# tho-kn/EgoTAP

Measured on AMD Instinct MI355X. Metric: stereo frames/sec (2D->3D lift, B=256, 256x256), higher is better.
Workload: dtype f32; 1 GPU; UnrealEgo 16-joint lifting head (heatmaps [B,90,64,64] -> joints [B,16,3]), forward only, fp32, batch 256 per GPU, inputs resident in HBM; batch_per_gpu=256, global_batch=256, heatmap=64, parallelism=dp1 (batch shards, no collective)

## Files before the change

egotap_amd/csrc/attention_f32.h:

```cpp
#pragma once
#include "common.h"
#include <math.h>
#ifdef EGOTAP_ATTN_F32_OLD
#include "../../tools/experiments/attention_f32_r2.h"
#else

template <int NW>
struct AttnCfg {
    static constexpr int DH = 128, KT = 32, KLD = DH + 4, THREADS = 64 * NW;
    static constexpr int TILE_FLOATS = KT * KLD + KT * DH;
    static constexpr int OUT_FLOATS = NW * 32 * KLD;
    static constexpr int LDS_BYTES = 4 * (TILE_FLOATS > OUT_FLOATS ? TILE_FLOATS : OUT_FLOATS);
};

template <int NW>
__global__ __launch_bounds__(64 * NW, 2) void attention_f32_kernel(const float* __restrict__ QKV,
                                                                 float* __restrict__ CTX, int N, int heads,
                                                                 int qgroups, float scale_log2e, float* __restrict__ LSE, int ksplit) {
    using Cfg = AttnCfg<NW>;
    constexpr int DH = Cfg::DH, KT = Cfg::KT, KLD = Cfg::KLD, THREADS = Cfg::THREADS;
    extern __shared__ __attribute__((aligned(16))) float smem[];
    float* Ks = smem;
    float* Vs = smem + KT * KLD;

    const int nblk = gridDim.x, bid = blockIdx.x;
    const int q8 = nblk >> 3, r8 = nblk & 7, x8 = bid & 7;
    const int lin = (x8 < r8 ? x8 * (q8 + 1) : r8 * (q8 + 1) + (x8 - r8) * q8) + (bid >> 3);
    const int split = ksplit > 1 ? lin % ksplit : 0;
    const int lq = ksplit > 1 ? lin / ksplit : lin;
    const int bh = lq / qgroups, qg = lq - bh * qgroups;
    const int b = bh / heads, h = bh - b * heads;

    const int tid = threadIdx.x, lane = tid & 63, wid = tid >> 6;
    const int l31 = lane & 31, lh = lane >> 5;
    const int D = heads * DH;
    const long ld = 3L * D;
    const float* base = QKV + (long)b * N * ld + h * DH;
    const int qb = qg * NW + wid;
    const bool valid = qb * 32 < N;
    const int q0 = min(qb * 32, N - 32);

    float qreg[64];
    {
        const float* qp = base + (long)(q0 + l31) * ld + 4 * lh;
#pragma unroll
        for (int t = 0; t < 16; ++t) {
            const f32x4 v = *(const f32x4*)(qp + 8 * t);
            qreg[4 * t + 0] = v[0]; qreg[4 * t + 1] = v[1]; qreg[4 * t + 2] = v[2]; qreg[4 * t + 3] = v[3];
        }
    }
    float m_run = -INFINITY, l_run = 0.f;

    constexpr int PER = KT * (DH / 4) / THREADS;
    f32x4 stg[PER];
    auto tile_req = [&](int kt, int vpart) __attribute__((always_inline)) {
        const float* kp = base + (long)min(kt * KT, N - KT) * ld + D + vpart * D;
#pragma unroll
        for (int i = 0; i < PER; ++i) {
            const int idx = tid + i * THREADS, row = idx >> 5, c4 = idx & 31;
            stg[i] = *(const f32x4*)(kp + (size_t)(unsigned)(row * (int)ld + c4 * 4));
        }
    };
    auto tile_put = [&](int vpart) __attribute__((always_inline)) {
#pragma unroll
        for (int i = 0; i < PER; ++i) {
            const int idx = tid + i * THREADS, row = idx >> 5, c4 = idx & 31;
            if (vpart) *(f32x4*)(Vs + row * DH + c4 * 4) = stg[i];
// ... 73 lines not shown
                s[r] = __builtin_amdgcn_exp2f(fmaf(s[r], scale_log2e, -m_run));
                psum += s[r];
            }
            l_run += psum;
#pragma unroll
            for (int r = 0; r < 16; ++r) {
                const float* vf = Vs + ((r & 3) + 8 * (r >> 2) + 4 * lh) * DH + l31;
#pragma unroll
                for (int dt = 0; dt < 4; ++dt)
                    o[dt] = __builtin_amdgcn_mfma_f32_32x32x2f32(vf[dt * 32], s[r], o[dt], 0, 0, 0);
            }
        }
        __syncthreads();
        if (kt + 1 < ntiles) {
            tile_put(1);
            if (kt + 2 < ntiles) tile_req(kt + 2, 0);
        }
    }
    __syncthreads();
    if (valid) {
        const float l_tot = l_run + __shfl_xor(l_run, 32, 64);
        const float inv = 1.0f / l_tot;
        const long part = ksplit > 1 ? (long)split * (gridDim.x / (ksplit * qgroups)) : 0;
        if (LSE != nullptr && lh == 0) LSE[(part + (long)b * heads + h) * N + q0 + l31] = m_run * 0.6931471805599453f + logf(l_tot);
        float* Os = smem + wid * 32 * KLD;
#pragma unroll
        for (int dt = 0; dt < 4; ++dt)
#pragma unroll
            for (int g = 0; g < 4; ++g) {
                f32x4 v;
#pragma unroll
                for (int c = 0; c < 4; ++c) v[c] = o[dt][4 * g + c] * inv;
                *(f32x4*)(Os + l31 * KLD + dt * 32 + 8 * g + 4 * lh) = v;
            }
        float* out = CTX + (part / heads * N + (long)b * N + q0) * D + h * DH;
#pragma unroll
        for (int it = 0; it < 16; ++it) {
            const int row = it * 2 + lh;
            const f32x4 v = *(const f32x4*)(Os + row * KLD + l31 * 4);
            *(f32x4*)(out + (long)row * D + l31 * 4) = v;
        }
    }
}

static __global__ __launch_bounds__(256) void attention_f32_merge_kernel(const float* __restrict__ part, const float* __restrict__ lse_part, float* __restrict__ ctx,
                                                                         int B, int N, int heads, int ksplit) {
    const long i = (long)blockIdx.x * blockDim.x + threadIdx.x;
    const long total = (long)B * N * heads * 32;
    if (i >= total) return;
    const int c4 = (int)(i & 31);
    const long t = i >> 5;
    const int h = (int)(t % heads);
    const long bn = t / heads;
    const int b = (int)(bn / N), n = (int)(bn - (long)b * N);
    float l[8], m = -INFINITY;
    for (int sp = 0; sp < ksplit; ++sp) {
        l[sp] = lse_part[(((long)sp * B + b) * heads + h) * N + n];
        m = fmaxf(m, l[sp]);
    }
    float wsum = 0.f;
    for (int sp = 0; sp < ksplit; ++sp) {
        l[sp] = expf(l[sp] - m);
        wsum += l[sp];
    }
    const float inv = 1.0f / wsum;
    f32x4 acc{0.f, 0.f, 0.f, 0.f};
    const long D = (long)heads * 128, off = bn * D + h * 128 + c4 * 4;
    for (int sp = 0; sp < ksplit; ++sp) {
        const f32x4 v = *(const f32x4*)(part + (long)sp * B * N * D + off);
        const float w = l[sp] * inv;
        acc[0] += w * v[0]; acc[1] += w * v[1]; acc[2] += w * v[2]; acc[3] += w * v[3];
    }
    *(f32x4*)(ctx + off) = acc;
}

static hipError_t attention_f32_launch(const float* QKV, float* CTX, int B, int N, int heads, hipStream_t stream,
                                       float* LSE = nullptr, float* scratch = nullptr, size_t scratch_floats = 0, int num_cu = 256) {
    constexpr int NW = 2;
    using Cfg = AttnCfg<NW>;
    if (B <= 0) return hipSuccess;
    if (N < 32 || N % 4 != 0) return hipErrorInvalidValue;
    auto kern = attention_f32_kernel<NW>;
    const int qgroups = ((N + 31) / 32 + NW - 1) / NW;
    const float scale_log2e = 1.4426950408889634f / sqrtf(128.0f);
    const long wgs = (long)B * heads * qgroups;
    int ksplit = 1;
    if (scratch != nullptr && LSE == nullptr) {
        const int ntiles = (N + 31) / 32;
        for (int k = 8; k >= 2; --k)
            if (ntiles % k == 0 && wgs * k <= 9L * num_cu / 2 && (size_t)k * ((size_t)B * N * heads * 128 + (size_t)B * heads * N) <= scratch_floats) { ksplit = k; break; }
    }
    if (ksplit > 1) {
        float* part = scratch;
        float* lse_part = scratch + (size_t)ksplit * B * N * heads * 128;
        hipLaunchKernelGGL(kern, dim3((unsigned)(wgs * ksplit)), dim3(Cfg::THREADS), Cfg::LDS_BYTES, stream, QKV, part, N, heads, qgroups, scale_log2e, lse_part, ksplit);
        hipError_t e = hipGetLastError();
        if (e != hipSuccess) return e;
        const long total = (long)B * N * heads * 32;
        hipLaunchKernelGGL(attention_f32_merge_kernel, dim3((unsigned)((total + 255) / 256)), dim3(256), 0, stream, (const float*)part, (const float*)lse_part, CTX, B, N, heads, ksplit);
        return hipGetLastError();
    }
    hipLaunchKernelGGL(kern, dim3(B * heads * qgroups), dim3(Cfg::THREADS), Cfg::LDS_BYTES, stream, QKV, CTX, N, heads,
                       qgroups, scale_log2e, LSE, 1);
    return hipGetLastError();
}
#endif
```

egotap_amd/csrc/egotap_abi.hip:

```cpp
#include <stdarg.h>
#include <stdio.h>
#include <string.h>

#include <string>
#include <unordered_map>
#include <vector>

#include "attention_f32.h"
#include "common.h"
#include "conv_f32.h"
#include "conv_bf16.h"
#include "gemm_f32.h"
#include "gemm_bf16.h"
#include "gemm_bf16_dma.h"
#include "gemm_f32_dma.h"
#include "attention_bf16.h"
#include "layernorm.h"
#include "metrics.h"
#include "heatmap_synth.h"
#include "pu_chain.h"
#include "gemm_tn_bf16.h"
#include "train_ops.h"
#include "gemm_bf16s.h"
#include "gemm_bf16s64.h"
// ... 407 lines not shown
    GemmTimer(Handle* h_, hipStream_t s_, const char* role, const char* kernel, double flops)
        : h(h_), s(s_), on(h_ && h_->timing) {
        if (!on) return;
        if (h->ev_used + 2 > h->ev.size()) {
            hipEvent_t a, b;
            if (hipEventCreate(&a) != hipSuccess || hipEventCreate(&b) != hipSuccess) { on = false; return; }
            h->ev.push_back(a);
            h->ev.push_back(b);
        }
        (void)hipEventRecord(h->ev[h->ev_used], s);
        h->rec.push_back({role, kernel, flops});
    }
    ~GemmTimer() {
        if (!on) return;
        (void)hipEventRecord(h->ev[h->ev_used + 1], s);
        h->ev_used += 2;
    }
};

template <class AL> struct AlName;
template <> struct AlName<ALoadPlain> { static constexpr const char* v = "ALoadPlain"; };
template <> struct AlName<ALoadPatch> { static constexpr const char* v = "ALoadPatch"; };
template <> struct AlName<ALoadTokens> { static constexpr const char* v = "ALoadTokens"; };
template <> struct AlName<ALoadRot> { static constexpr const char* v = "ALoadRot"; };
template <> struct AlName<ALoadStereo> { static constexpr const char* v = "ALoadStereo"; };
template <> struct AlName<ALoadStereoGated> { static constexpr const char* v = "ALoadStereoGated"; };
template <class E> struct EpiName;
template <> struct EpiName<EpiBias> { static constexpr const char* v = "EpiBias"; };
template <> struct EpiName<EpiBiasRes> { static constexpr const char* v = "EpiBiasRes"; };
template <> struct EpiName<EpiBiasGelu> { static constexpr const char* v = "EpiBiasGelu"; };
template <> struct EpiName<EpiBnLrelu> { static constexpr const char* v = "EpiBnLrelu"; };
template <> struct EpiName<EpiPatch> { static constexpr const char* v = "EpiPatch"; };

template <class Cfg, class AL, class Epi>
static hipError_t gemm(Handle* h, const char* role, const AL& al, const SegMat& W, const Epi& epi, float* C, long ldc,
                       int M, int N, int K, hipStream_t s) {
    static const std::string kname = std::string("gemm_f32_kernel<") + std::to_string(Cfg::BM) + "x" +
                                     std::to_string(Cfg::BN) + "x" + std::to_string(Cfg::BK) + "," + AlName<AL>::v + "," +
                                     EpiName<Epi>::v + ">";
    GemmTimer t(h, s, role, kname.c_str(), 2.0 * M * N * K);
    return gemm_f32_launch<Cfg, AL, Epi>(al, W, epi, C, ldc, M, N, K, s);
}

static int device_cu_count() {
    static int n = 0;
    if (n == 0) {
        int dev = 0, v = 0;
        if (hipGetDevice(&dev) == hipSuccess && hipDeviceGetAttribute(&v, hipDeviceAttributeMultiprocessorCount, dev) == hipSuccess && v > 0) n = v;
        else n = 256;
    }
    return n;
}
// ... 317 lines not shown
}

#if EGOTAP_IN(0)
static hipError_t gemm_res_ln(Handle* h, const char* role, const float* A, long lda, const float* Wp, const float* bias, float* X, int M, int D, int K,
                              const float* ln_g, const float* ln_b, float* Y, float* P, hipStream_t s) {
    if (D == 1024) {
        const SmallRoute r = gemm_small_route(h, true, M, D, K, D, device_cu_count());
        if ((r.kind == GS_SPLIT_S || r.kind == GS_SPLIT_A) && r.splits > 1) {
            static const std::string kname = "gemm_f32_splitk_kernel<ALoadPlain>+splitk_reduce_res_ln_kernel";
            GemmTimer t(h, s, role, kname.c_str(), 2.0 * M * D * K);
            hipError_t e = r.kind == GS_SPLIT_S ? gemm_f32_splitk_partials<TileS>(ALoadPlain{A, lda}, segmat1(Wp, D, K), P, SPLITK_FLOATS, M, D, K, s, r.splits)
                                                : gemm_f32_splitk_partials<TileA>(ALoadPlain{A, lda}, segmat1(Wp, D, K), P, SPLITK_FLOATS, M, D, K, s, r.splits);
            if (e != hipSuccess) return e;
            hipLaunchKernelGGL(splitk_reduce_res_ln_kernel<1024>, dim3(min((M + 3) / 4, 256 * 8)), dim3(256), 0, s, (const float*)P, bias, (const float*)X, X, ln_g,
                               ln_b, Y, M, r.splits, 1e-12f);
            return hipGetLastError();
        }
    }
    hipError_t e = gemm_small(h, role, ALoadPlain{A, lda}, segmat1(Wp, D, K), EpiBiasRes{segvec1(bias, D), X, D}, X, D, M, D, K, P, s);
    if (e != hipSuccess) return e;
    return launch_ln(X, Y, ln_g, ln_b, M, 1e-12f, s);
}

extern "C" int egotap_lift_forward(egotap_handle h, const float* hm, int B, float* pose, void* ws, size_t ws_bytes,
                                   void* stream) {
    EGO_CHECK(h, "null handle");
    if (B == 0) return EGOTAP_OK;
    EGO_CHECK(B > 0 && hm && pose && ws, "egotap_lift_forward: null argument or negative batch");
    EGO_CHECK(((uintptr_t)hm & 15) == 0 && ((uintptr_t)ws & 255) == 0, "hm must be 16-byte and ws 256-byte aligned");
    int rc = lift_resolve(h);
    if (rc != EGOTAP_OK) return rc;
    const LiftWs w = lift_ws(h, B);
    if (ws_bytes < w.total) {
        egotap_set_error("workspace too small: %zu bytes given, %zu needed for B=%d", ws_bytes, w.total, B);
        return EGOTAP_ERR_WORKSPACE;
    }
    hipStream_t s = (hipStream_t)stream;
    const LiftParams& p = h->lp;
    char* base = (char*)ws;
    auto F = [&](size_t off) { return (float*)(base + off); };
    float *X = F(w.X), *Y = F(w.Y), *QKV = F(w.QKV), *CTX = F(w.CTX), *HID = F(w.HID);
    float* SPK = F(w.SPLITK);
    float *Z1 = F(w.Z1), *Z2 = F(w.Z2), *POSZ = F(w.POSZ), *ROTZ = F(w.ROTZ);
    float *F0 = F(w.F0), *G0 = F(w.G0), *HS0 = F(w.HS0), *F1 = F(w.F1), *G1 = F(w.G1), *HS1 = F(w.HS1);
    float *C0 = F(w.C0), *C1 = F(w.C1), *ZERO = F(w.ZERO), *HPA = F(w.HPA), *HPB = F(w.HPB);
    const int D = h->D, M = B * h->seq, BT = B * h->T, J = h->J, H = h->H, hid = h->hid, JB = J * B;
    const int S = h->cfg.hm_size, HW = S * S;
    using Tile = TileA;

#ifndef EGOTAP_BF16S_MIN_ROWS
#define EGOTAP_BF16S_MIN_ROWS 512
// ... 55 lines not shown
            prep(p.pos_fc[0].w, Wb, 2048, K1);
            const XTokens xt{Yb, h->T, D, h->seq, h->side, h->ppd, h->grid};
            const int sp = gemm_bf16s_ksplit(BT, 2048, K1, cu, SPLITK_FLOATS);
            if (sp > 1) EGO_HIP(gemm_bf16s_splitk_launch(xt, Wb, (long)K1, bnf(p.pos_fc[0], Z1), SPK, sp, BT, 2048, K1, cu, s));
            else EGO_HIP(fc1_nt(h, 0, Yb, Wb, (long)K1, bnf(p.pos_fc[0], Z1), BT, cu, s));
            EGO_HIP((fc_gemm(h, "pos_fc2", ALoadPlain{Z1, 2048}, segmat1(p.pos_fc[1].w, 512, 2048), bn(p.pos_fc[1]), Z2, 512, BT, 512, 2048, SPK, s)));
            EGO_HIP((fc_gemm(h, "pos_fc3", ALoadPlain{Z2, 512}, segmat1(p.pos_fc[2].w, hid, 512), bn(p.pos_fc[2]), POSZ, hid, BT, hid, 512, SPK, s)));
        }
        {
            __bf16* hmb = HIDb;
            const long n8 = (long)B * h->C * HW / 8;
            hipLaunchKernelGGL(f32_to_bf16_kernel, dim3((unsigned)((n8 + 255) / 256)), dim3(256), 0, s, hm, hmb, n8);
            prep(p.rot_fc[0].w, Wb, 2048, 2 * HW);
            EGO_HIP(hipGetLastError());
            const XRot xr{hmb, h->C, J, HW};
            const int sp = gemm_bf16s_ksplit(BT, 2048, 2 * HW, cu, SPLITK_FLOATS);
            if (sp > 1) EGO_HIP(gemm_bf16s_splitk_launch(xr, Wb, 2L * HW, bnf(p.rot_fc[0], Z1), SPK, sp, BT, 2048, 2 * HW, cu, s));
            else EGO_HIP(fc1_nt(h, 1, hmb, Wb, 2L * HW, bnf(p.rot_fc[0], Z1), BT, cu, s));
            EGO_HIP((fc_gemm(h, "rot_fc2", ALoadPlain{Z1, 2048}, segmat1(p.rot_fc[1].w, 512, 2048), bn(p.rot_fc[1]), Z2, 512, BT, 512, 2048, SPK, s)));
            EGO_HIP((fc_gemm(h, "rot_fc3", ALoadPlain{Z2, 512}, segmat1(p.rot_fc[2].w, hid, 512), bn(p.rot_fc[2]), ROTZ, hid, BT, hid, 512, SPK, s)));
        }
    } else {
    const int NL = h->cfg.vit_layers;
    EGO_HIP(launch_ln(X, Y, NL > 0 ? p.layer[0].ln1_g : p.lnf_g, NL > 0 ? p.layer[0].ln1_b : p.lnf_b, M, 1e-12f, s));
    for (int i = 0; i < NL; ++i) {
        const auto& L = p.layer[i];
        {
            SegMat Wqkv; Wqkv.p[0] = L.q_w; Wqkv.p[1] = L.k_w; Wqkv.p[2] = L.v_w; Wqkv.seg = D; Wqkv.ld = D;
            SegVec bqkv; bqkv.p[0] = L.q_b; bqkv.p[1] = L.k_b; bqkv.p[2] = L.v_b; bqkv.seg = D;
            EGO_HIP((gemm_small(h, "qkv", ALoadPlain{Y, D}, Wqkv, EpiBias{bqkv}, QKV, 3L * D, M, 3 * D, D, SPK, s)));
        }
        if (h->precision == EGOTAP_PREC_BF16X3 && h->seq % 32 == 0) EGO_HIP(attention_bf16_launch<3>(QKV, CTX, B, h->seq, h->cfg.vit_heads, s));
        else if (h->precision == EGOTAP_PREC_BF16 && h->seq % 32 == 0) EGO_HIP(attention_bf16_launch<1>(QKV, CTX, B, h->seq, h->cfg.vit_heads, s));
        else EGO_HIP(attention_f32_launch(QKV, CTX, B, h->seq, h->cfg.vit_heads, s, nullptr, SPK, SPLITK_FLOATS, device_cu_count()));
        EGO_HIP(gemm_res_ln(h, "attn_out", CTX, D, L.o_w, L.o_b, X, M, D, D, L.ln2_g, L.ln2_b, Y, SPK, s));
        EGO_HIP((gemm_small(h, "mlp_up", ALoadPlain{Y, D}, segmat1(L.up_w, 4 * D, D), EpiBiasGelu{segvec1(L.up_b, 4 * D)}, HID, 4L * D, M, 4 * D, D, SPK, s)));
        const bool last = i + 1 == NL;
        EGO_HIP(gemm_res_ln(h, "mlp_down", HID, 4L * D, L.dn_w, L.dn_b, X, M, D, 4 * D, last ? p.lnf_g : p.layer[i + 1].ln1_g, last ? p.lnf_b : p.layer[i + 1].ln1_b, Y,
                            SPK, s));
        if (h->debug_stop == 2 + i) return EGOTAP_OK;
    }
    auto bn = [](const LiftParams::Fc& f) { return EpiBnLrelu{f.b, f.g, f.beta, f.mean, f.var, 1e-5f, 0.2f}; };
    const bool skinny_fc1 = BT < SKINNY_ROWS || (h->precision == EGOTAP_PREC_F32 && (long)((BT + 255) / 256) * (2048 / 256) < 100);
    {
        const int K1 = h->ppd * h->ppd * D;
        ALoadTokens al{Y, h->T, D, h->seq, h->side, h->ppd, h->grid};
        if (skinny_fc1 && BT <= 64)
            EGO_HIP((gemm_f32_splitk_launch<TileS>(al, segmat1(p.pos_fc[0].w, 2048, K1), bn(p.pos_fc[0]), Z1, 2048, SPK, SPLITK_FLOATS, BT, 2048, K1, s, device_cu_count())));
        else if (skinny_fc1)
            EGO_HIP((gemm_f32_splitk_launch<TileA>(al, segmat1(p.pos_fc[0].w, 2048, K1), bn(p.pos_fc[0]), Z1, 2048, SPK, SPLITK_FLOATS, BT, 2048, K1, s)));
        else
            EGO_HIP((gemm_big(h, "pos_fc1", al, segmat1(p.pos_fc[0].w, 2048, K1), bn(p.pos_fc[0]), Z1, 2048, BT, 2048, K1, s)));
        EGO_HIP((fc_gemm(h, "pos_fc2", ALoadPlain{Z1, 2048}, segmat1(p.pos_fc[1].w, 512, 2048), bn(p.pos_fc[1]), Z2, 512, BT, 512, 2048, SPK, s)));
        EGO_HIP((fc_gemm(h, "pos_fc3", ALoadPlain{Z2, 512}, segmat1(p.pos_fc[2].w, hid, 512), bn(p.pos_fc[2]), POSZ, hid, BT, hid, 512, SPK, s)));
    }
    {
        ALoadRot al{hm, h->C, J, HW};
        if (skinny_fc1 && BT <= 64)
            EGO_HIP((gemm_f32_splitk_launch<TileS>(al, segmat1(p.rot_fc[0].w, 2048, 2L * HW), bn(p.rot_fc[0]), Z1, 2048, SPK, SPLITK_FLOATS, BT, 2048, 2 * HW, s, device_cu_count())));
        else if (skinny_fc1)
            EGO_HIP((gemm_f32_splitk_launch<TileA>(al, segmat1(p.rot_fc[0].w, 2048, 2L * HW), bn(p.rot_fc[0]), Z1, 2048, SPK, SPLITK_FLOATS, BT, 2048, 2 * HW, s)));
        else
            EGO_HIP((gemm_big(h, "rot_fc1", al, segmat1(p.rot_fc[0].w, 2048, 2L * HW), bn(p.rot_fc[0]), Z1, 2048, BT, 2048, 2 * HW, s)));
        EGO_HIP((fc_gemm(h, "rot_fc2", ALoadPlain{Z1, 2048}, segmat1(p.rot_fc[1].w, 512, 2048), bn(p.rot_fc[1]), Z2, 512, BT, 512, 2048, SPK, s)));
        EGO_HIP((fc_gemm(h, "rot_fc3", ALoadPlain{Z2, 512}, segmat1(p.rot_fc[2].w, hid, 512), bn(p.rot_fc[2]), ROTZ, hid, BT, hid, 512, SPK, s)));
    }
    }
    const int x = 2 * hid, NF0 = H + x;
    ALoadStereo xs{POSZ, B, J, hid};
    EGO_HIP((fc_gemm(h, "pu0_x2f", xs, segmat1(p.x2f0_w, NF0, x), EpiBias{segvec1(p.x2f0_b, NF0)}, F0, NF0, JB, NF0, x, SPK, s)));
    EGO_HIP((fc_gemm(h, "pu0_x2h", xs, segmat1(p.x2h0_w, 4 * H, x), EpiBias{segvec1(p.x2h0_b, 4 * H)}, G0, 4L * H, JB, 4 * H, x, SPK, s)));
    {
        ALoadStereoGated bs{ALoadStereo{ROTZ, B, J, hid}, F0, NF0, H};
        EGO_HIP((fc_gemm(h, "pu0_b2h", bs, segmat1(p.b2h0_w, 4 * H, x), EpiBiasRes{segvec1(p.b2h0_b, 4 * H), G0, 4L * H}, G0, 4L * H, JB, 4 * H, x, SPK, s)));
    }
// ... 4 lines not shown
                      FAULT, h->pu_fault_dev};
    if (!pu_chain_launch(s, h->pu_resident[0], h->pu_resident[1], ch0, B, h->pu_debug_drop))
    for (int t = 0; t < J; ++t) {
        const float* hp_in = t == 0 ? ZERO : ((t & 1) ? HPA : HPB);
        pu_step_launch(s, B, H, hp_in, G0 + (size_t)t * B * 4 * H, p.h2h0_w, p.h2h0_b, C0, C0, HS0 + (size_t)t * B * H,
                       t + 1 < J ? F0 + (size_t)(t + 1) * B * NF0 : nullptr, NF0, (t & 1) ? HPB : HPA, nullptr);
    }
    EGO_HIP(hipGetLastError());
    EGO_HIP((fc_gemm(h, "pu1_x2f", ALoadPlain{HS0, H}, segmat1(p.x2f1_w, H, H), EpiBias{segvec1(p.x2f1_b, H)}, F1, H, JB, H, H, SPK, s)));
    EGO_HIP((fc_gemm(h, "pu1_x2h", ALoadPlain{HS0, H}, segmat1(p.x2h1_w, 4 * H, H), EpiBias{segvec1(p.x2h1_b, 4 * H)}, G1, 4L * H, JB, 4 * H, H, SPK, s)));
    const PuChain ch1{F1, (long)B * H, H, G1, (long)B * 4 * H, nullptr, p.h2h1_w, p.h2h1_b, nullptr, 0, HS1, (long)B * H, HPA, (long)B * H, B, H, J,
                      FAULT, h->pu_fault_dev};
    if (!pu_chain_launch(s, h->pu_resident[0], h->pu_resident[1], ch1, B, h->pu_debug_drop))
    for (int t = 0; t < J; ++t) {
        const float* hp_in = t == 0 ? ZERO : ((t & 1) ? HPA : HPB);
        pu_step_launch(s, B, H, hp_in, G1 + (size_t)t * B * 4 * H, p.h2h1_w, p.h2h1_b, C1, C1, HS1 + (size_t)t * B * H,
                       t + 1 < J ? F1 + (size_t)(t + 1) * B * H : nullptr, H, (t & 1) ? HPB : HPA, nullptr);
    }
    EGO_HIP(hipGetLastError());
    hipLaunchKernelGGL(pose_head_kernel, dim3(B, h->J + 1), dim3(256), 0, s, POSZ, HS1, p.pose_w, p.pose_b, p.glob_w, p.glob_b, pose, B,
                       J, hid, H, h->cfg.estimate_head);
    EGO_HIP(hipGetLastError());
    return EGOTAP_OK;
}
#endif

static int hm_resolve(Handle* h, int net) {
    if (h->hm_resolved[net]) return EGOTAP_OK;
    bool ok = true;
    HmParams& p = h->hp[net];
    const std::string bb = "backbone.backbone.backbone.";
    auto bn = [&](const std::string& k) {
        auto n = h->bound[net].find(k + ".num_batches_tracked");
        long long* nbt = (n != h->bound[net].end() && n->second.dtype == EGOTAP_I64 && n->second.numel == 1) ? (long long*)n->second.ptr : nullptr;
        return HmParams::Bn{P(h, net, k + ".weight", ok), P(h, net, k + ".bias", ok), P(h, net, k + ".running_mean", ok),
                            P(h, net, k + ".running_var", ok), nbt};
    };
    p.stem_w = P(h, net, bb + "conv1.weight", ok);
    p.stem_bn = bn(bb + "bn1");
    for (int i = 0; i < 4; ++i) p.nblk[i] = hm_nblk(h, i);
    for (int i = 0; i < 4; ++i)
        for (int b = 0; b < p.nblk[i]; ++b) {
            const std::string k = bb + "layer" + std::to_string(i + 1) + "." + std::to_string(b);
            auto& B = p.blk[i][b];
            B.w1 = P(h, net, k + ".conv1.weight", ok); B.bn1 = bn(k + ".bn1");
            B.w2 = P(h, net, k + ".conv2.weight", ok); B.bn2 = bn(k + ".bn2");
// ... 2416 lines not shown
```

egotap_amd/csrc/gemm_f32.h:

```cpp
#pragma once
#include "common.h"
#include <type_traits>

struct ALoadPlain {
    const float* A;
    long lda;
    struct Row { const float* p; };
    __device__ __forceinline__ Row row(int m) const { return Row{A + (long)m * lda}; }
    __device__ __forceinline__ f32x4 load(const Row& r, int k) const { return *(const f32x4*)(r.p + k); }
    static constexpr bool HAS_PTR = true;
    __device__ __forceinline__ const float* ptr(const Row& r, int k) const { return r.p + k; }
    __host__ bool dma_ok() const { return lda % 4 == 0 && lda < (1L << 21) && ((uintptr_t)A & 15) == 0; }
};

struct ALoadPatch {
    const float* hm;
    int C, S, seq, side, ppd, grid, T;
    const float* zeros = nullptr;
    struct Row { const float* p; };
    static constexpr bool HAS_PTR = true;
    __device__ __forceinline__ const float* ptr(const Row& r, int k) const { return r.p ? r.p + (k >> 4) * S + (k & 15) : zeros + k; }
    __host__ bool dma_ok() const { return zeros != nullptr && S % 4 == 0 && ((uintptr_t)hm & 15) == 0 && ((uintptr_t)zeros & 15) == 0; }
    __device__ __forceinline__ Row row(int m) const {
        const int b = m / seq, tok = m - b * seq;
// ... 10 lines not shown

struct ALoadTokens {
    const float* Y;
    int T, D, seq, side, ppd, grid;
    struct Row { const float* p; };
    __device__ __forceinline__ Row row(int m) const {
        const int b = m / T, i = m - b * T;
        return Row{Y + ((long)b * seq + (long)(ppd * (i / grid)) * side + ppd * (i % grid)) * D};
    }
    __device__ __forceinline__ f32x4 load(const Row& r, int k) const {
        const int s = k / D, c = k - s * D;
        const int prl = s / ppd, pcl = s - prl * ppd;
        return *(const f32x4*)(r.p + (long)(prl * side + pcl) * D + c);
    }
    static constexpr bool HAS_PTR = true;
    __device__ __forceinline__ const float* ptr(const Row& r, int k) const {
        const int s = k / D, c = k - s * D;
        const int prl = s / ppd, pcl = s - prl * ppd;
        return r.p + (long)(prl * side + pcl) * D + c;
    }
    __host__ bool dma_ok() const { return D % 4 == 0 && ((uintptr_t)Y & 15) == 0; }
};

struct ALoadRot {
    const float* hm;
    int C, J, HW;
    struct Row { const float* p; };
    __device__ __forceinline__ Row row(int m) const {
        const int T = 2 * J;
        const int b = m / T, t = m - b * T;
        const int eye = t / J, j = t - eye * J;
        return Row{hm + (long)(b * C + 2 * J + eye * 2 * J + j) * HW};
    }
    __device__ __forceinline__ f32x4 load(const Row& r, int k) const {
        const int cs = k / HW;
        return *(const f32x4*)(r.p + (long)cs * J * HW + (k - cs * HW));
    }
    static constexpr bool HAS_PTR = true;
    __device__ __forceinline__ const float* ptr(const Row& r, int k) const {
        const int cs = k / HW;
        return r.p + (long)cs * J * HW + (k - cs * HW);
    }
    __host__ bool dma_ok() const { return HW % 4 == 0 && ((uintptr_t)hm & 15) == 0; }
};

struct ALoadStereo {
// ... 31 lines not shown
    SegVec bias;
    struct Col { float b; };
    __device__ __forceinline__ Col col(int n) const { return Col{bias.at(n)}; }
    __device__ __forceinline__ float apply(float acc, const Col& c, int m, int n) const { return acc + c.b; }
    struct Col4 { f32x4 b; };
    __device__ __forceinline__ Col4 col4(int n0) const { return Col4{bias.at4(n0)}; }
    static constexpr bool HAS_RES = false;
    __device__ __forceinline__ f32x4 res4(int m, int n0) const { return f32x4{0.f, 0.f, 0.f, 0.f}; }
    __device__ __forceinline__ f32x4 apply4(f32x4 acc, const Col4& c, f32x4 res, int m, int n0) const { return acc + c.b; }
};
struct EpiBiasRes {
    SegVec bias;
    const float* R;
    long ldr;
    struct Col { float b; };
    __device__ __forceinline__ Col col(int n) const { return Col{bias.at(n)}; }
    __device__ __forceinline__ float apply(float acc, const Col& c, int m, int n) const {
        return acc + c.b + R[(long)m * ldr + n];
    }
    struct Col4 { f32x4 b; };
    __device__ __forceinline__ Col4 col4(int n0) const { return Col4{bias.at4(n0)}; }
    static constexpr bool HAS_RES = true;
    __device__ __forceinline__ f32x4 res4(int m, int n0) const { return *(const f32x4*)(R + (long)m * ldr + n0); }
    __device__ __forceinline__ f32x4 apply4(f32x4 acc, const Col4& c, f32x4 res, int m, int n0) const { return acc + c.b + res; }
};
struct EpiBiasGelu {
    SegVec bias;
    struct Col { float b; };
    __device__ __forceinline__ Col col(int n) const { return Col{bias.at(n)}; }
    __device__ __forceinline__ float apply(float acc, const Col& c, int m, int n) const {
        const float x = acc + c.b;
        return gelu_erf(x);
    }
    struct Col4 { f32x4 b; };
    __device__ __forceinline__ Col4 col4(int n0) const { return Col4{bias.at4(n0)}; }
    static constexpr bool HAS_RES = false;
    __device__ __forceinline__ f32x4 res4(int m, int n0) const { return f32x4{0.f, 0.f, 0.f, 0.f}; }
    __device__ __forceinline__ f32x4 apply4(f32x4 acc, const Col4& c, f32x4 res, int m, int n0) const {
        f32x4 o;
#pragma unroll
        for (int i = 0; i < 4; ++i) {
            const float x = acc[i] + c.b[i];
            o[i] = gelu_erf(x);
        }
        return o;
    }
// ... 762 lines not shown
```

egotap_amd/lib.py:

```python
from __future__ import annotations

import ctypes as C
import os

from . import build as _build

ERR_NAMES = {1: "EGOTAP_ERR_INVALID", 2: "EGOTAP_ERR_HIP", 3: "EGOTAP_ERR_UNBOUND", 4: "EGOTAP_ERR_WORKSPACE"}
NET_LIFT, NET_HM_POS, NET_HM_ROT = 0, 1, 2
F32, I64 = 0, 1
PRECISIONS = {"f32": 0, "bf16x3": 1, "bf16": 2}


class EgotapConfig(C.Structure):
    _fields_ = [(n, C.c_int32) for n in (
        "struct_bytes", "n_joints_hm", "estimate_head", "hm_size", "hidden", "vit_dim", "vit_heads", "vit_layers",
        "patch", "pu_hidden")] + [("hm_blocks", C.c_int32 * 4)]


class EgotapError(RuntimeError):
    pass


_lib = None

_PROTOS = {
    "egotap_abi_version": (C.c_int, []),
    "egotap_last_error": (C.c_char_p, []),
    "egotap_create": (C.c_int, [C.POINTER(EgotapConfig), C.POINTER(C.c_void_p)]),
    "egotap_destroy": (None, [C.c_void_p]),
    "egotap_bind_param": (C.c_int, [C.c_void_p, C.c_int, C.c_char_p, C.c_void_p, C.c_int64, C.c_int]),
    "egotap_unbound_count": (C.c_int, [C.c_void_p, C.c_int, C.POINTER(C.c_int)]),
    "egotap_lift_workspace_bytes": (C.c_int, [C.c_void_p, C.c_int, C.POINTER(C.c_size_t)]),
    "egotap_lift_forward": (C.c_int, [C.c_void_p, C.c_void_p, C.c_int, C.c_void_p, C.c_void_p, C.c_size_t, C.c_void_p]),
    "egotap_lift_intermediate": (C.c_int, [C.c_void_p, C.c_int, C.c_char_p, C.POINTER(C.c_size_t), C.POINTER(C.c_int64)]),
    "egotap_lift_debug_stop": (C.c_int, [C.c_void_p, C.c_int]),
    "egotap_set_precision": (C.c_int, [C.c_void_p, C.c_int]),
    "egotap_set_pu_chain": (C.c_int, [C.c_void_p, C.c_int]),
    "egotap_pu_chain_status": (C.c_int, [C.c_void_p, C.POINTER(C.c_int), C.POINTER(C.c_int)]),
    "egotap_debug_pu_drop_workgroups": (C.c_int, [C.c_void_p, C.c_int]),
    "egotap_debug_gemm_bk": (C.c_int, [C.c_int]),
    "egotap_debug_conv_addressing": (C.c_int, [C.c_int]),
    "egotap_set_weight_scratch": (C.c_int, [C.c_void_p, C.c_void_p, C.c_size_t]),
    "egotap_set_act_scratch": (C.c_int, [C.c_void_p, C.c_void_p, C.c_size_t]),
    "egotap_hm_workspace_bytes": (C.c_int, [C.c_void_p, C.c_int, C.POINTER(C.c_size_t)]),
    "egotap_hm_forward": (C.c_int, [C.c_void_p, C.c_int, C.c_void_p, C.c_void_p, C.c_int, C.c_void_p, C.c_int64, C.c_void_p,
                                    C.c_size_t, C.c_void_p]),
    "egotap_hm_intermediate": (C.c_int, [C.c_void_p, C.c_int, C.c_char_p, C.POINTER(C.c_size_t), C.POINTER(C.c_int64)]),
    "egotap_hm_forward_bnbatch_workspace_bytes": (C.c_int, [C.c_void_p, C.c_int, C.c_int, C.POINTER(C.c_size_t)]),
    "egotap_hm_forward_bnbatch_intermediate": (C.c_int, [C.c_void_p, C.c_int, C.c_int, C.c_char_p, C.POINTER(C.c_size_t), C.POINTER(C.c_int64)]),
    "egotap_hm_forward_bnbatch": (C.c_int, [C.c_void_p, C.c_int, C.c_void_p, C.c_void_p, C.c_int, C.c_void_p, C.c_int64, C.c_int, C.c_void_p,
                                            C.c_size_t, C.c_void_p]),
    "egotap_linear_f32": (C.c_int, [C.c_void_p] * 4 + [C.c_int] * 4 + [C.c_void_p] * 5 + [C.c_int, C.c_void_p]),
    "egotap_gemm_tile_name": (C.c_char_p, [C.c_int]),
    "egotap_linear_bf16_dma": (C.c_int, [C.c_void_p] * 4 + [C.c_int] * 3 + [C.c_void_p]),
    "egotap_layernorm_f32": (C.c_int, [C.c_void_p] * 4 + [C.c_int, C.c_int, C.c_float, C.c_void_p]),
    "egotap_attention_f32": (C.c_int, [C.c_void_p, C.c_void_p, C.c_int, C.c_int, C.c_int, C.c_void_p]),
# ... 219 lines not shown
```

egotap_amd/networks.py:

```python
from __future__ import annotations

import ctypes as C
import os

import torch
import torch.nn as nn

from . import lib as _lib
from . import spec as _spec


class _Node(nn.Module):

    def forward(self, *a, **k):
        raise RuntimeError("parameter container: compute happens in libegotap_hip.so")


def _build_tree(root: nn.Module, entries):
    for key, shape in entries:
        parts = key.split(".")
        mod = root
        for p in parts[:-1]:
            if p not in mod._modules:
                mod.add_module(p, _Node())
# ... 159 lines not shown
        return self.forward(input, input_rgb_left, input_rgb_right, pose_only=True)

    def forward(self, input, input_rgb_left=None, input_rgb_right=None, pose_only=False):
        p = self.preset
        if not input.is_cuda:
            raise _lib.EgotapError("EgoTAPAutoEncoder runs on the GPU only (no CPU fallback); move the input to cuda")
        if input.dim() != 4 or input.shape[1] != p.in_channels or input.shape[2] != p.hm_size or input.shape[3] != p.hm_size:
            raise ValueError(f"expected input [B, {p.in_channels}, {p.hm_size}, {p.hm_size}], got {tuple(input.shape)}")
        if self.training:
            from .training import lift_train_forward
            pose = lift_train_forward(self, input)
            return pose if pose_only else (pose,) + self._zero_outputs(input.shape[0], input.device)[1:]
        hm = input.detach()
        if hm.dtype != torch.float32:
            hm = hm.float()
        hm = hm.contiguous()
        B = hm.shape[0]
        dev = hm.device
        pose = torch.empty((B, p.out_joints, 3), dtype=torch.float32, device=dev)
        if B > 0:
            with torch.cuda.device(dev):
                self._bind(dev)
                ws = self._workspace(B, dev)
                _lib.check(_lib.load().egotap_lift_forward(
                    self._ensure_handle(), C.c_void_p(hm.data_ptr()), B, C.c_void_p(pose.data_ptr()),
                    C.c_void_p(ws.data_ptr()), ws.numel(), C.c_void_p(torch.cuda.current_stream(dev).cuda_stream)))
        if pose_only:
            return pose
        return (pose,) + self._zero_outputs(B, dev)[1:]

    def predict_pose_graphed(self, input):
        if self.training:
            raise RuntimeError("predict_pose_graphed is an inference path: call .eval() first")
        p = self.preset
        if not input.is_cuda:
            raise _lib.EgotapError("EgoTAPAutoEncoder runs on the GPU only (no CPU fallback); move the input to cuda")
        if input.dim() != 4 or tuple(input.shape[1:]) != (p.in_channels, p.hm_size, p.hm_size):
            raise ValueError(f"expected input [B, {p.in_channels}, {p.hm_size}, {p.hm_size}], got {tuple(input.shape)}")
        dev = input.device
        self._bind(dev)
        B = input.shape[0]
        key = (B, str(dev), getattr(self, "precision", "f32"), self._bound_sig)
        graphs = self.__dict__.setdefault("_graphs", {})
        g = graphs.get(key)
        if g is None:
            lib, h = _lib.load(), self._ensure_handle()
            static_in = input.detach().float().contiguous().clone()
            static_out = torch.empty((B, p.out_joints, 3), dtype=torch.float32, device=dev)
            self.predict_pose(static_in)
            need = C.c_size_t()
            _lib.check(lib.egotap_lift_workspace_bytes(h, B, C.byref(need)))
            ws = torch.empty(need.value, dtype=torch.uint8, device=dev)
            self._act_scratch(B, dev)
            keep = (ws, getattr(self, "_ascratch", None), getattr(self, "_wscratch", None))

            def run():
                _lib.check(lib.egotap_lift_forward(h, C.c_void_p(static_in.data_ptr()), B, C.c_void_p(static_out.data_ptr()),
                                                   C.c_void_p(ws.data_ptr()), ws.numel(), C.c_void_p(torch.cuda.current_stream(dev).cuda_stream)))
            side = torch.cuda.Stream(dev)
            side.wait_stream(torch.cuda.current_stream(dev))
            with torch.cuda.device(dev), torch.cuda.stream(side):
                run()
            torch.cuda.current_stream(dev).wait_stream(side)
            graph = torch.cuda.CUDAGraph()
            with torch.cuda.device(dev), torch.cuda.graph(graph, stream=side):
                run()
            if len(graphs) >= 8:
                graphs.pop(next(iter(graphs)))
            g = graphs[key] = (graph, static_in, static_out, keep)
        graph, static_in, static_out, _ = g
        static_in.copy_(input)
        graph.replay()
        return static_out

    def _zero_outputs(self, B, dev):
        p = self.preset
        key = (B, str(dev))
        if key not in self._zeros:
            z = torch.zeros((), dtype=torch.float32, device=dev)
            self._zeros = {key: (torch.zeros((B, self.rot_dim), device=dev), torch.zeros((B, 6 * p.n_joints_hm), device=dev),
                                 z.expand(B, p.in_channels, p.hm_size, p.hm_size))}
# ... 295 lines not shown
```

include/egotap.h:

```cpp
#ifndef EGOTAP_H
#define EGOTAP_H
#include <stddef.h>
#include <stdint.h>

#ifdef __cplusplus
extern "C" {
#endif

#define EGOTAP_ABI_VERSION 2

enum { EGOTAP_OK = 0, EGOTAP_ERR_INVALID = 1, EGOTAP_ERR_HIP = 2, EGOTAP_ERR_UNBOUND = 3, EGOTAP_ERR_WORKSPACE = 4 };

enum { EGOTAP_NET_LIFT = 0, EGOTAP_NET_HM_POS = 1, EGOTAP_NET_HM_ROT = 2, EGOTAP_NET_COUNT = 3 };

enum { EGOTAP_F32 = 0, EGOTAP_I64 = 1 };

typedef struct egotap_config {
    int32_t struct_bytes;
    int32_t n_joints_hm;
    int32_t estimate_head;
    int32_t hm_size;
    int32_t hidden;
    int32_t vit_dim;
    int32_t vit_heads;
    int32_t vit_layers;
    int32_t patch;
    int32_t pu_hidden;
    int32_t hm_blocks[4];
} egotap_config;

typedef struct egotap_handle_s* egotap_handle;

int egotap_abi_version(void);
const char* egotap_last_error(void);

int egotap_create(const egotap_config* cfg, egotap_handle* out);
void egotap_destroy(egotap_handle h);

int egotap_bind_param(egotap_handle h, int net, const char* state_dict_key, void* dev_ptr, int64_t numel, int dtype);
int egotap_unbound_count(egotap_handle h, int net, int* count);

int egotap_lift_workspace_bytes(egotap_handle h, int B, size_t* bytes);
int egotap_lift_forward(egotap_handle h, const float* hm, int B, float* pose, void* ws, size_t ws_bytes, void* stream);

int egotap_lift_intermediate(egotap_handle h, int B, const char* name, size_t* offset, int64_t* numel);

int egotap_hm_workspace_bytes(egotap_handle h, int B, size_t* bytes);
int egotap_hm_forward(egotap_handle h, int net, const float* left, const float* right, int B, float* out,
                      int64_t out_image_stride, void* ws, size_t ws_bytes, void* stream);
int egotap_hm_intermediate(egotap_handle h, int B, const char* name, size_t* offset, int64_t* numel);
int egotap_hm_forward_bnbatch_workspace_bytes(egotap_handle h, int B, int chunk, size_t* bytes);
int egotap_hm_forward_bnbatch(egotap_handle h, int net, const float* left, const float* right, int B, float* out, int64_t out_image_stride,
                              int chunk, void* ws, size_t ws_bytes, void* stream);
int egotap_hm_forward_bnbatch_intermediate(egotap_handle h, int B, int chunk, const char* name, size_t* offset, int64_t* numel);

enum { EGOTAP_PREC_F32 = 0, EGOTAP_PREC_BF16X3 = 1, EGOTAP_PREC_BF16 = 2 };
int egotap_set_precision(egotap_handle h, int mode);
int egotap_set_pu_chain(egotap_handle h, int enable);
int egotap_pu_chain_status(egotap_handle h, int* enabled, int* faults);
int egotap_set_weight_scratch(egotap_handle h, void* buf, size_t bytes);
int egotap_set_act_scratch(egotap_handle h, void* buf, size_t bytes);


int egotap_linear_f32(const float* x, const float* w, const float* b, float* y, int M, int N, int K, int epi,
                      const float* r, const float* bn_gamma, const float* bn_beta, const float* bn_mean,
                      const float* bn_var, int tile, void* stream);
// ... 125 lines not shown
```

Before: 2773 stereo frames/s.

## Prune last ViT layer to live token rows in pose-only lift path

Adds a pose-only entry point that computes the last transformer layer's Q projection, attention, output projection, LN and MLP only for the token rows the pose FC head consumes. K/V are still computed for every row. The attention kernel gains a separate query source, stride and query count, and new gather-style A-loader and residual epilogue types map compact rows back to their physical positions. A cost-model-based split of each GEMM into full rounds plus a remainder is also added. The work is semantically equivalent for pose output, but it adds indexing overhead and intermediate activations are no longer full.

```diff
diff --git a/egotap_amd/csrc/attention_f32.h b/egotap_amd/csrc/attention_f32.h
--- a/egotap_amd/csrc/attention_f32.h
+++ b/egotap_amd/csrc/attention_f32.h
@@ -4,6 +4,7 @@
 #ifdef EGOTAP_ATTN_F32_OLD
 #include "../../tools/experiments/attention_f32_r2.h"
 #else
+#define EGOTAP_ATTN_F32_LIVE 1
 
 template <int NW>
 struct AttnCfg {
@@ -16,7 +17,8 @@
 template <int NW>
 __global__ __launch_bounds__(64 * NW, 2) void attention_f32_kernel(const float* __restrict__ QKV,
                                                                  float* __restrict__ CTX, int N, int heads,
-                                                                 int qgroups, float scale_log2e, float* __restrict__ LSE, int ksplit) {
+                                                                 int qgroups, float scale_log2e, float* __restrict__ LSE, int ksplit,
+                                                                 const float* __restrict__ Qsrc, long ldq, int Nq) {
     using Cfg = AttnCfg<NW>;
     constexpr int DH = Cfg::DH, KT = Cfg::KT, KLD = Cfg::KLD, THREADS = Cfg::THREADS;
     extern __shared__ __attribute__((aligned(16))) float smem[];
@@ -37,12 +39,12 @@
     const long ld = 3L * D;
     const float* base = QKV + (long)b * N * ld + h * DH;
     const int qb = qg * NW + wid;
-    const bool valid = qb * 32 < N;
-    const int q0 = min(qb * 32, N - 32);
+    const bool valid = qb * 32 < Nq;
+    const int q0 = min(qb * 32, Nq - 32);
 
     float qreg[64];
     {
-        const float* qp = base + (long)(q0 + l31) * ld + 4 * lh;
+        const float* qp = Qsrc + ((long)b * Nq + q0 + l31) * ldq + h * DH + 4 * lh;
 #pragma unroll
         for (int t = 0; t < 16; ++t) {
             const f32x4 v = *(const f32x4*)(qp + 8 * t);
@@ -162,7 +164,7 @@
         const float l_tot = l_run + __shfl_xor(l_run, 32, 64);
         const float inv = 1.0f / l_tot;
         const long part = ksplit > 1 ? (long)split * (gridDim.x / (ksplit * qgroups)) : 0;
-        if (LSE != nullptr && lh == 0) LSE[(part + (long)b * heads + h) * N + q0 + l31] = m_run * 0.6931471805599453f + logf(l_tot);
+        if (LSE != nullptr && lh == 0) LSE[(part + (long)b * heads + h) * Nq + q0 + l31] = m_run * 0.6931471805599453f + logf(l_tot);
         float* Os = smem + wid * 32 * KLD;
 #pragma unroll
         for (int dt = 0; dt < 4; ++dt)
@@ -173,7 +175,7 @@
                 for (int c = 0; c < 4; ++c) v[c] = o[dt][4 * g + c] * inv;
                 *(f32x4*)(Os + l31 * KLD + dt * 32 + 8 * g + 4 * lh) = v;
             }
-        float* out = CTX + (part / heads * N + (long)b * N + q0) * D + h * DH;
+        float* out = CTX + (part / heads * Nq + (long)b * Nq + q0) * D + h * DH;
 #pragma unroll
         for (int it = 0; it < 16; ++it) {
             const int row = it * 2 + lh;
@@ -214,6 +216,14 @@
     *(f32x4*)(ctx + off) = acc;
 }
 
+static int attention_f32_ksplit(int B, int N, int heads, size_t scratch_floats, int num_cu) {
+    const long wgs = (long)B * heads * (((N + 31) / 32 + 1) / 2);
+    const int ntiles = (N + 31) / 32;
+    for (int k = 8; k >= 2; --k)
+        if (ntiles % k == 0 && wgs * k <= 9L * num_cu / 2 && (size_t)k * ((size_t)B * N * heads * 128 + (size_t)B * heads * N) <= scratch_floats) return k;
+    return 1;
+}
+
 static hipError_t attention_f32_launch(const float* QKV, float* CTX, int B, int N, int heads, hipStream_t stream,
                                        float* LSE = nullptr, float* scratch = nullptr, size_t scratch_floats = 0, int num_cu = 256) {
     constexpr int NW = 2;
@@ -224,16 +234,12 @@
     const int qgroups = ((N + 31) / 32 + NW - 1) / NW;
     const float scale_log2e = 1.4426950408889634f / sqrtf(128.0f);
     const long wgs = (long)B * heads * qgroups;
-    int ksplit = 1;
-    if (scratch != nullptr && LSE == nullptr) {
-        const int ntiles = (N + 31) / 32;
-        for (int k = 8; k >= 2; --k)
-            if (ntiles % k == 0 && wgs * k <= 9L * num_cu / 2 && (size_t)k * ((size_t)B * N * heads * 128 + (size_t)B * heads * N) <= scratch_floats) { ksplit = k; break; }
-    }
+    const int ksplit = scratch != nullptr && LSE == nullptr ? attention_f32_ksplit(B, N, heads, scratch_floats, num_cu) : 1;
     if (ksplit > 1) {
         float* part = scratch;
         float* lse_part = scratch + (size_t)ksplit * B * N * heads * 128;
-        hipLaunchKernelGGL(kern, dim3((unsigned)(wgs * ksplit)), dim3(Cfg::THREADS), Cfg::LDS_BYTES, stream, QKV, part, N, heads, qgroups, scale_log2e, lse_part, ksplit);
+        hipLaunchKernelGGL(kern, dim3((unsigned)(wgs * ksplit)), dim3(Cfg::THREADS), Cfg::LDS_BYTES, stream, QKV, part, N, heads, qgroups, scale_log2e, lse_part, ksplit,
+                           QKV, 3L * heads * Cfg::DH, N);
         hipError_t e = hipGetLastError();
         if (e != hipSuccess) return e;
         const long total = (long)B * N * heads * 32;
@@ -241,7 +247,19 @@
         return hipGetLastError();
     }
     hipLaunchKernelGGL(kern, dim3(B * heads * qgroups), dim3(Cfg::THREADS), Cfg::LDS_BYTES, stream, QKV, CTX, N, heads,
-                       qgroups, scale_log2e, LSE, 1);
+                       qgroups, scale_log2e, LSE, 1, QKV, 3L * heads * Cfg::DH, N);
     return hipGetLastError();
 }
+
+static hipError_t attention_f32_live_launch(const float* Q, long ldq, int Nq, const float* QKV, float* CTX, int B, int N, int heads, hipStream_t stream) {
+    constexpr int NW = 2;
+    using Cfg = AttnCfg<NW>;
+    if (B <= 0) return hipSuccess;
+    if (N < 32 || N % 4 != 0 || Nq < 32 || Nq > N || ldq % 4 != 0) return hipErrorInvalidValue;
+    const int qgroups = ((Nq + 31) / 32 + NW - 1) / NW;
+    const float scale_log2e = 1.4426950408889634f / sqrtf(128.0f);
+    hipLaunchKernelGGL(attention_f32_kernel<NW>, dim3(B * heads * qgroups), dim3(Cfg::THREADS), Cfg::LDS_BYTES, stream, QKV, CTX, N, heads,
+                       qgroups, scale_log2e, (float*)nullptr, 1, Q, ldq, Nq);
+    return hipGetLastError();
+}
 #endif
diff --git a/egotap_amd/csrc/egotap_abi.hip b/egotap_amd/csrc/egotap_abi.hip
--- a/egotap_amd/csrc/egotap_abi.hip
+++ b/egotap_amd/csrc/egotap_abi.hip
@@ -453,12 +453,14 @@
 template <> struct AlName<ALoadPlain> { static constexpr const char* v = "ALoadPlain"; };
 template <> struct AlName<ALoadPatch> { static constexpr const char* v = "ALoadPatch"; };
 template <> struct AlName<ALoadTokens> { static constexpr const char* v = "ALoadTokens"; };
+template <> struct AlName<ALoadLive> { static constexpr const char* v = "ALoadLive"; };
 template <> struct AlName<ALoadRot> { static constexpr const char* v = "ALoadRot"; };
 template <> struct AlName<ALoadStereo> { static constexpr const char* v = "ALoadStereo"; };
 template <> struct AlName<ALoadStereoGated> { static constexpr const char* v = "ALoadStereoGated"; };
 template <class E> struct EpiName;
 template <> struct EpiName<EpiBias> { static constexpr const char* v = "EpiBias"; };
 template <> struct EpiName<EpiBiasRes> { static constexpr const char* v = "EpiBiasRes"; };
+template <> struct EpiName<EpiBiasResLive> { static constexpr const char* v = "EpiBiasResLive"; };
 template <> struct EpiName<EpiBiasGelu> { static constexpr const char* v = "EpiBiasGelu"; };
 template <> struct EpiName<EpiBnLrelu> { static constexpr const char* v = "EpiBnLrelu"; };
 template <> struct EpiName<EpiPatch> { static constexpr const char* v = "EpiPatch"; };
@@ -822,11 +824,51 @@
     return launch_ln(X, Y, ln_g, ln_b, M, 1e-12f, s);
 }
 
-extern "C" int egotap_lift_forward(egotap_handle h, const float* hm, int B, float* pose, void* ws, size_t ws_bytes,
-                                   void* stream) {
+static ALoadPlain rebase(const ALoadPlain& a, int m0) { return ALoadPlain{a.A + (long)m0 * a.lda, a.lda}; }
+static ALoadLive rebase(ALoadLive a, int m0) { a.lr.m0 += m0; return a; }
+static EpiBias rebase(const EpiBias& e, int) { return e; }
+static EpiBiasGelu rebase(const EpiBiasGelu& e, int) { return e; }
+static EpiBiasRes rebase(EpiBiasRes e, int m0) { e.R += (long)m0 * e.ldr; return e; }
+static EpiBiasResLive rebase(EpiBiasResLive e, int m0) { e.lr.m0 += m0; return e; }
+template <class AL, class Epi>
+static hipError_t gemm_rounds(Handle* h, const char* role, const AL& al, const SegMat& W, const Epi& epi, float* C, long ldc, int M, int N, int K,
+                              hipStream_t s) {
+    const int cus = device_cu_count(), tn = N / 256;
+    const long tiles = (long)((M + 255) / 256) * tn;
+    const int mh = (int)((tiles / cus) * cus / tn) * 256;
+    if (N % 256 == 0 && K % 32 == 0 && mh > 0 && mh < M) {
+        const double t_round = K * 0.2319 + 5.0;
+        const double t_big = (double)((tiles + cus - 1) / cus) * t_round;
+        const double t_split = (double)(((long)(mh / 256) * tn + cus - 1) / cus) * t_round + 4.0 + gemm_f32_direct_estimate_us<TileA>(M - mh, N, K, cus);
+        if (t_split < t_big) {
+            hipError_t e = gemm_big(h, role, al, W, epi, C, ldc, mh, N, K, s);
+            if (e != hipSuccess) return e;
+            return gemm<TileA>(h, role, rebase(al, mh), W, rebase(epi, mh), C + (long)mh * ldc, ldc, M - mh, N, K, s);
+        }
+    }
+    return gemm_big(h, role, al, W, epi, C, ldc, M, N, K, s);
+}
+
+static bool lift_prune_last(Handle* h, int B) {
+#ifdef EGOTAP_ATTN_F32_LIVE
+    const int D = h->D, M = B * h->seq, Nq = h->T * h->ppd * h->ppd;
+    if (h->precision != EGOTAP_PREC_F32 || h->debug_stop != 0 || h->cfg.vit_layers < 1 || Nq < 32 || Nq >= h->seq || D % 256 != 0) return false;
+    const int cus = device_cu_count();
+    if (gemm_small_route(h, true, M, 3 * D, D, D, cus, true).kind != GS_BIG || gemm_small_route(h, true, M, D, D, D, cus).kind != GS_BIG ||
+        gemm_small_route(h, true, M, 4 * D, D, 4 * D, cus, true).kind != GS_BIG || gemm_small_route(h, true, M, D, 4 * D, D, cus).kind != GS_BIG)
+        return false;
+    return attention_f32_ksplit(B, h->seq, h->cfg.vit_heads, SPLITK_FLOATS, cus) == 1;
+#else
+    (void)h; (void)B;
+    return false;
+#endif
+}
+
+static int lift_forward_impl(Handle* h, const float* hm, int B, float* pose, void* ws, size_t ws_bytes, void* stream, bool pose_only,
+                             const char* who) {
     EGO_CHECK(h, "null handle");
     if (B == 0) return EGOTAP_OK;
-    EGO_CHECK(B > 0 && hm && pose && ws, "egotap_lift_forward: null argument or negative batch");
+    EGO_CHECK(B > 0 && hm && pose && ws, "%s: null argument or negative batch", who);
     EGO_CHECK(((uintptr_t)hm & 15) == 0 && ((uintptr_t)ws & 255) == 0, "hm must be 16-byte and ws 256-byte aligned");
     int rc = lift_resolve(h);
     if (rc != EGOTAP_OK) return rc;
@@ -928,9 +970,28 @@
         }
     } else {
     const int NL = h->cfg.vit_layers;
+    const bool prune = pose_only && lift_prune_last(h, B);
     EGO_HIP(launch_ln(X, Y, NL > 0 ? p.layer[0].ln1_g : p.lnf_g, NL > 0 ? p.layer[0].ln1_b : p.lnf_b, M, 1e-12f, s));
     for (int i = 0; i < NL; ++i) {
         const auto& L = p.layer[i];
+#ifdef EGOTAP_ATTN_F32_LIVE
+        if (prune && i + 1 == NL) {
+            const LiveRows lr{h->seq, h->side, h->ppd, h->grid, h->T};
+            const int Nq = h->T * h->ppd * h->ppd, Mc = B * Nq;
+            float* Xc = QKV;
+            SegMat Wkv; Wkv.p[0] = L.k_w; Wkv.p[1] = L.v_w; Wkv.p[2] = L.v_w; Wkv.seg = D; Wkv.ld = D;
+            SegVec bkv; bkv.p[0] = L.k_b; bkv.p[1] = L.v_b; bkv.p[2] = L.v_b; bkv.seg = D;
+            EGO_HIP((gemm_big(h, "kv", ALoadPlain{Y, D}, Wkv, EpiBias{bkv}, QKV + D, 3L * D, M, 2 * D, D, s)));
+            EGO_HIP((gemm_rounds(h, "q_live", ALoadLive{Y, D, lr}, segmat1(L.q_w, D, D), EpiBias{segvec1(L.q_b, D)}, QKV, 3L * D, Mc, D, D, s)));
+            EGO_HIP(attention_f32_live_launch(QKV, 3L * D, Nq, QKV, CTX, B, h->seq, h->cfg.vit_heads, s));
+            EGO_HIP((gemm_rounds(h, "attn_out_live", ALoadPlain{CTX, D}, segmat1(L.o_w, D, D), EpiBiasResLive{segvec1(L.o_b, D), X, D, lr}, Xc, D, Mc, D, D, s)));
+            EGO_HIP(launch_ln(Xc, Y, L.ln2_g, L.ln2_b, Mc, 1e-12f, s));
+            EGO_HIP((gemm_rounds(h, "mlp_up_live", ALoadPlain{Y, D}, segmat1(L.up_w, 4 * D, D), EpiBiasGelu{segvec1(L.up_b, 4 * D)}, HID, 4L * D, Mc, 4 * D, D, s)));
+            EGO_HIP((gemm_rounds(h, "mlp_down_live", ALoadPlain{HID, 4L * D}, segmat1(L.dn_w, D, 4 * D), EpiBiasRes{segvec1(L.dn_b, D), Xc, D}, Xc, D, Mc, D, 4 * D, s)));
+            EGO_HIP(launch_ln(Xc, Y, p.lnf_g, p.lnf_b, Mc, 1e-12f, s));
+            break;
+        }
+#endif
         {
             SegMat Wqkv; Wqkv.p[0] = L.q_w; Wqkv.p[1] = L.k_w; Wqkv.p[2] = L.v_w; Wqkv.seg = D; Wqkv.ld = D;
             SegVec bqkv; bqkv.p[0] = L.q_b; bqkv.p[1] = L.k_b; bqkv.p[2] = L.v_b; bqkv.seg = D;
@@ -950,13 +1011,15 @@
     const bool skinny_fc1 = BT < SKINNY_ROWS || (h->precision == EGOTAP_PREC_F32 && (long)((BT + 255) / 256) * (2048 / 256) < 100);
     {
         const int K1 = h->ppd * h->ppd * D;
-        ALoadTokens al{Y, h->T, D, h->seq, h->side, h->ppd, h->grid};
-        if (skinny_fc1 && BT <= 64)
-            EGO_HIP((gemm_f32_splitk_launch<TileS>(al, segmat1(p.pos_fc[0].w, 2048, K1), bn(p.pos_fc[0]), Z1, 2048, SPK, SPLITK_FLOATS, BT, 2048, K1, s, device_cu_count())));
-        else if (skinny_fc1)
-            EGO_HIP((gemm_f32_splitk_launch<TileA>(al, segmat1(p.pos_fc[0].w, 2048, K1), bn(p.pos_fc[0]), Z1, 2048, SPK, SPLITK_FLOATS, BT, 2048, K1, s)));
-        else
-            EGO_HIP((gemm_big(h, "pos_fc1", al, segmat1(p.pos_fc[0].w, 2048, K1), bn(p.pos_fc[0]), Z1, 2048, BT, 2048, K1, s)));
+        auto fc1 = [&](const auto& al) -> hipError_t {
+            if (skinny_fc1 && BT <= 64)
+                return gemm_f32_splitk_launch<TileS>(al, segmat1(p.pos_fc[0].w, 2048, K1), bn(p.pos_fc[0]), Z1, 2048, SPK, SPLITK_FLOATS, BT, 2048, K1, s, device_cu_count());
+            if (skinny_fc1)
+                return gemm_f32_splitk_launch<TileA>(al, segmat1(p.pos_fc[0].w, 2048, K1), bn(p.pos_fc[0]), Z1, 2048, SPK, SPLITK_FLOATS, BT, 2048, K1, s);
+            return gemm_big(h, "pos_fc1", al, segmat1(p.pos_fc[0].w, 2048, K1), bn(p.pos_fc[0]), Z1, 2048, BT, 2048, K1, s);
+        };
+        if (prune) EGO_HIP(fc1(ALoadPlain{Y, (long)K1}));
+        else EGO_HIP(fc1(ALoadTokens{Y, h->T, D, h->seq, h->side, h->ppd, h->grid}));
         EGO_HIP((fc_gemm(h, "pos_fc2", ALoadPlain{Z1, 2048}, segmat1(p.pos_fc[1].w, 512, 2048), bn(p.pos_fc[1]), Z2, 512, BT, 512, 2048, SPK, s)));
         EGO_HIP((fc_gemm(h, "pos_fc3", ALoadPlain{Z2, 512}, segmat1(p.pos_fc[2].w, hid, 512), bn(p.pos_fc[2]), POSZ, hid, BT, hid, 512, SPK, s)));
     }
@@ -1007,6 +1070,13 @@
                        J, hid, H, h->cfg.estimate_head);
     EGO_HIP(hipGetLastError());
     return EGOTAP_OK;
+}
+
+extern "C" int egotap_lift_forward(egotap_handle h, const float* hm, int B, float* pose, void* ws, size_t ws_bytes, void* stream) {
+    return lift_forward_impl(h, hm, B, pose, ws, ws_bytes, stream, false, "egotap_lift_forward");
+}
+extern "C" int egotap_lift_predict_pose(egotap_handle h, const float* hm, int B, float* pose, void* ws, size_t ws_bytes, void* stream) {
+    return lift_forward_impl(h, hm, B, pose, ws, ws_bytes, stream, true, "egotap_lift_predict_pose");
 }
 #endif
 
diff --git a/egotap_amd/csrc/gemm_f32.h b/egotap_amd/csrc/gemm_f32.h
--- a/egotap_amd/csrc/gemm_f32.h
+++ b/egotap_amd/csrc/gemm_f32.h
@@ -56,6 +56,29 @@
     __host__ bool dma_ok() const { return D % 4 == 0 && ((uintptr_t)Y & 15) == 0; }
 };
 
+struct LiveRows {
+    int seq, side, ppd, grid, T;
+    int m0 = 0;
+    __host__ __device__ __forceinline__ long phys(int m) const {
+        m += m0;
+        const int pp = ppd * ppd, L = T * pp;
+        const int b = m / L, r = m - b * L, i = r / pp, s = r - i * pp;
+        const int pr = (i / grid) * ppd + s / ppd, pc = (i % grid) * ppd + s % ppd;
+        return (long)b * seq + pr * side + pc;
+    }
+};
+struct ALoadLive {
+    const float* A;
+    long lda;
+    LiveRows lr;
+    struct Row { const float* p; };
+    __device__ __forceinline__ Row row(int m) const { return Row{A + lr.phys(m) * lda}; }
+    __device__ __forceinline__ f32x4 load(const Row& r, int k) const { return *(const f32x4*)(r.p + k); }
+    static constexpr bool HAS_PTR = true;
+    __device__ __forceinline__ const float* ptr(const Row& r, int k) const { return r.p + k; }
+    __host__ bool dma_ok() const { return lda % 4 == 0 && lda < (1L << 21) && ((uintptr_t)A & 15) == 0; }
+};
+
 struct ALoadRot {
     const float* hm;
     int C, J, HW;
@@ -133,6 +156,22 @@
     __device__ __forceinline__ Col4 col4(int n0) const { return Col4{bias.at4(n0)}; }
     static constexpr bool HAS_RES = true;
     __device__ __forceinline__ f32x4 res4(int m, int n0) const { return *(const f32x4*)(R + (long)m * ldr + n0); }
+    __device__ __forceinline__ f32x4 apply4(f32x4 acc, const Col4& c, f32x4 res, int m, int n0) const { return acc + c.b + res; }
+};
+struct EpiBiasResLive {
+    SegVec bias;
+    const float* R;
+    long ldr;
+    LiveRows lr;
+    struct Col { float b; };
+    __device__ __forceinline__ Col col(int n) const { return Col{bias.at(n)}; }
+    __device__ __forceinline__ float apply(float acc, const Col& c, int m, int n) const {
+        return acc + c.b + R[lr.phys(m) * ldr + n];
+    }
+    struct Col4 { f32x4 b; };
+    __device__ __forceinline__ Col4 col4(int n0) const { return Col4{bias.at4(n0)}; }
+    static constexpr bool HAS_RES = true;
+    __device__ __forceinline__ f32x4 res4(int m, int n0) const { return *(const f32x4*)(R + lr.phys(m) * ldr + n0); }
     __device__ __forceinline__ f32x4 apply4(f32x4 acc, const Col4& c, f32x4 res, int m, int n0) const { return acc + c.b + res; }
 };
 struct EpiBiasGelu {
diff --git a/egotap_amd/lib.py b/egotap_amd/lib.py
--- a/egotap_amd/lib.py
+++ b/egotap_amd/lib.py
@@ -32,6 +32,7 @@
     "egotap_unbound_count": (C.c_int, [C.c_void_p, C.c_int, C.POINTER(C.c_int)]),
     "egotap_lift_workspace_bytes": (C.c_int, [C.c_void_p, C.c_int, C.POINTER(C.c_size_t)]),
     "egotap_lift_forward": (C.c_int, [C.c_void_p, C.c_void_p, C.c_int, C.c_void_p, C.c_void_p, C.c_size_t, C.c_void_p]),
+    "egotap_lift_predict_pose": (C.c_int, [C.c_void_p, C.c_void_p, C.c_int, C.c_void_p, C.c_void_p, C.c_size_t, C.c_void_p]),
     "egotap_lift_intermediate": (C.c_int, [C.c_void_p, C.c_int, C.c_char_p, C.POINTER(C.c_size_t), C.POINTER(C.c_int64)]),
     "egotap_lift_debug_stop": (C.c_int, [C.c_void_p, C.c_int]),
     "egotap_set_precision": (C.c_int, [C.c_void_p, C.c_int]),
diff --git a/egotap_amd/networks.py b/egotap_amd/networks.py
--- a/egotap_amd/networks.py
+++ b/egotap_amd/networks.py
@@ -205,7 +205,8 @@
             with torch.cuda.device(dev):
                 self._bind(dev)
                 ws = self._workspace(B, dev)
-                _lib.check(_lib.load().egotap_lift_forward(
+                entry = _lib.load().egotap_lift_predict_pose if pose_only else _lib.load().egotap_lift_forward
+                _lib.check(entry(
                     self._ensure_handle(), C.c_void_p(hm.data_ptr()), B, C.c_void_p(pose.data_ptr()),
                     C.c_void_p(ws.data_ptr()), ws.numel(), C.c_void_p(torch.cuda.current_stream(dev).cuda_stream)))
         if pose_only:
@@ -238,8 +239,8 @@
             keep = (ws, getattr(self, "_ascratch", None), getattr(self, "_wscratch", None))
 
             def run():
-                _lib.check(lib.egotap_lift_forward(h, C.c_void_p(static_in.data_ptr()), B, C.c_void_p(static_out.data_ptr()),
-                                                   C.c_void_p(ws.data_ptr()), ws.numel(), C.c_void_p(torch.cuda.current_stream(dev).cuda_stream)))
+                _lib.check(lib.egotap_lift_predict_pose(h, C.c_void_p(static_in.data_ptr()), B, C.c_void_p(static_out.data_ptr()),
+                                                        C.c_void_p(ws.data_ptr()), ws.numel(), C.c_void_p(torch.cuda.current_stream(dev).cuda_stream)))
             side = torch.cuda.Stream(dev)
             side.wait_stream(torch.cuda.current_stream(dev))
             with torch.cuda.device(dev), torch.cuda.stream(side):
diff --git a/include/egotap.h b/include/egotap.h
--- a/include/egotap.h
+++ b/include/egotap.h
@@ -42,6 +42,7 @@
 
 int egotap_lift_workspace_bytes(egotap_handle h, int B, size_t* bytes);
 int egotap_lift_forward(egotap_handle h, const float* hm, int B, float* pose, void* ws, size_t ws_bytes, void* stream);
+int egotap_lift_predict_pose(egotap_handle h, const float* hm, int B, float* pose, void* ws, size_t ws_bytes, void* stream);
 
 int egotap_lift_intermediate(egotap_handle h, int B, const char* name, size_t* offset, int64_t* numel);
 
```

Result: faster. 2891 stereo frames/s (median of 6 runs) (+4.2%).
